# YihongSun/Dynamo-Depth

Hardware: AMD Instinct MI355X
Metric: training images/sec (192x640 triplets) (higher is better)
Workload: dtype f32

## Files before the change

dynamo-depth_amd/csrc/dd_conv_mfma.hip:

```cpp
#include <hip/hip_runtime.h>
#include <cstdlib>
#include <type_traits>

#include "../../include/dynamo_hip.h"
#include "dd_attr.h"
#include "dd_split.h"
#include "dd_store_tile.h"

namespace dd {
namespace cm {

constexpr int TH = 8, TW = 32, NT = 256;
constexpr int HH = TH + 2, HW = TW + 2, HN = HH * HW;
constexpr int CK = 16;
constexpr int PSTR = 48;
constexpr int A_PIECE = HN * PSTR;
constexpr int A_BYTES = 3 * A_PIECE;
__device__ __forceinline__ int halo_addr(int px, int half) {
  return px * 48 + half * 16;
}
__host__ __device__ constexpr int pieces_of(int products) { return products == 6 ? 3 : (products == 3 ? 2 : 1); }
constexpr int FRAG = 1024;
constexpr int PRE = (HN * 4 + NT - 1) / NT;

// ... 176 lines not shown
      if (tap == 1) fetch(min(chunk + 1, nchunks - 1));
      constexpr int PA[6] = {2, 0, 1, 1, 0, 0}, PB[6] = {0, 2, 1, 0, 1, 0};
#pragma unroll
      for (int t = 6 - NP; t < 6; ++t)
#pragma unroll
        for (int m = 0; m < 2; ++m)
#pragma unroll
          for (int n = 0; n < NB; ++n)
            acc[m][n] = __builtin_amdgcn_mfma_f32_32x32x16_bf16(__builtin_bit_cast(bf8, af[cur][m][PA[t]]), __builtin_bit_cast(bf8, bfr[cur][n][PB[t]]), acc[m][n], 0, 0, 0);
      __builtin_amdgcn_sched_barrier(0);
      if (tap < 8) {
        store_b(s + 2);
        lds_barrier();
      }
    }
  }

  auto tail = [&](auto full) {
#pragma unroll
    for (int n = 0; n < NB; ++n) {
      const int co = (ntile * NB + n) * 32 + (lane & 31);
#pragma unroll
      for (int m = 0; m < 2; ++m) {
        const int Y = Y0 + 2 * wave + m, X = X0 + 4 * (lane >> 5);
        float* p = y + (((size_t)b * Ho + Y) * Wo + X) * n_out + co;
        store_acc32<decltype(full)::value>(acc[m][n], bv[n], p, (size_t)n_out, (co < n_out && Y < Ho) ? Wo - X : 0, StoreF32{});
      }
    }
  };
  if (X0 + TW <= Wo && Y0 + TH <= Ho && (ntile + 1) * (32 * NB) <= n_out) tail(std::true_type{});
  else tail(std::false_type{});
}

constexpr int FLAT_MT = 256;
constexpr int FLAT_ZERO = HN - 1;
constexpr int FLAT_MAX_W = (FLAT_ZERO - FLAT_MT) / 2 - 1;

template <int NB, int NP>
__global__ __launch_bounds__(NT, 2) void conv_mfma_flat_kernel(const float* __restrict__ x, const uint4* __restrict__ pack, const float* __restrict__ bias,
                                                               int H, int W, int M, int k_in, int n_out, int splits, float* __restrict__ out) {
  extern __shared__ __align__(16) unsigned char smem[];
  unsigned char* const s_b = smem + A_BYTES;
  const int tid = threadIdx.x, lane = tid & 63, wave = __builtin_amdgcn_readfirstlane(tid >> 6);
  const int p0 = (int)blockIdx.x * FLAT_MT, ntile = blockIdx.y, split = blockIdx.z;
  const int nchunks = (k_in + CK - 1) / CK;
  const int c_begin = (int)((long long)nchunks * split / splits), c_end = (int)((long long)nchunks * (split + 1) / splits);
  const int win = FLAT_MT + 2 * (W + 1), q0 = p0 - (W + 1);
  const char* pk = reinterpret_cast<const char*>(pack) + (size_t)ntile * nchunks * 9 * (3 * NB * FRAG);

  int g_off[PRE], l_off[PRE];
#pragma unroll
  for (int j = 0; j < PRE; ++j) {
    const int i = tid + j * NT, px = i >> 2, q = i & 3;
    const int fp = q0 + px;
    l_off[j] = px < win ? halo_addr(px, q >> 1) + (q & 1) * 8 : -1;
    g_off[j] = (px < win && fp >= 0 && fp < M) ? fp * k_in + q * 4 : -1;
  }
  if (tid < 9) {
    const int pc = tid / 3, part = tid % 3;
    if (part * 16 < PSTR) *reinterpret_cast<uint4*>(smem + pc * A_PIECE + FLAT_ZERO * PSTR + part * 16) = make_uint4(0u, 0u, 0u, 0u);
  }
  float4 pre[PRE];
  auto fetch = [&](int chunk) {
#pragma unroll
    for (int j = 0; j < PRE; ++j) {
      const int c0 = chunk * CK + (((tid + j * NT) & 3) << 2);
// ... 136 lines not shown
    const float4 v = P[(size_t)s * total4 + i];
    a.x += v.x; a.y += v.y; a.z += v.z; a.w += v.w;
  }
  if (bias) {
    const int c = (i * 4) % n_out;
    a.x += bias[c]; a.y += bias[c + 1]; a.z += bias[c + 2]; a.w += bias[c + 3];
  }
  reinterpret_cast<float4*>(y)[i] = a;
}

static int flat_splits(int M, int k_in, int n_out) {
  const int wgs = ((M + FLAT_MT - 1) / FLAT_MT) * ((n_out + 63) / 64), nchunks = (k_in + CK - 1) / CK;
  const char* env = getenv("DD_FLAT_SPLITS");
  int s = env ? atoi(env) : (480 + wgs / 2) / wgs;
  if (s > nchunks / 2) s = nchunks / 2;
  return s < 1 ? 1 : s;
}

static size_t pack_bytes(int n_out, int k_in) { return (size_t)frags_of(n_out, k_in) * 3 * FRAG; }

template <int NB, int NP>
static int launch(const float* x, const void* pack, const float* bias, int B, int Hi, int Wi, int k_in, int n_out, int pad, float* y, hipStream_t stream) {
  const int Ho = Hi + 2 * pad - 2, Wo = Wi + 2 * pad - 2;
  const int tiles_x = (Wo + TW - 1) / TW, tiles_y = (Ho + TH - 1) / TH;
  auto kern = conv_mfma_kernel<NB, NP>;
  static dd::LdsAttrOnce lds_attr;
  if (const int rc = lds_attr.ensure(reinterpret_cast<const void*>(kern), (int)(lds_bytes<NB>()))) return rc;
  dim3 grid(tiles_x * tiles_y, (n_out + 32 * NB - 1) / (32 * NB), B);
  hipLaunchKernelGGL(kern, grid, dim3(NT), lds_bytes<NB>(), stream, x, static_cast<const uint4*>(pack), bias, Hi, Wi, Ho, Wo, k_in, n_out, pad, tiles_x,
                     tiles_y, y);
  return (int)hipGetLastError();
}

template <int NP>
static int launch_blocks(const float* x, const void* pack, const float* bias, int B, int Hi, int Wi, int k_in, int n_out, int pad, float* y, hipStream_t s) {
  switch (blocks_for(n_out)) {
    case 1: return launch<1, NP>(x, pack, bias, B, Hi, Wi, k_in, n_out, pad, y, s);
    case 2: return launch<2, NP>(x, pack, bias, B, Hi, Wi, k_in, n_out, pad, y, s);
    default: return launch<3, NP>(x, pack, bias, B, Hi, Wi, k_in, n_out, pad, y, s);
  }
}

template <int NP>
static int launch_flat(const float* x, const void* pack, const float* bias, int H, int W, int M, int k_in, int n_out, int splits, float* out, hipStream_t s) {
  auto kern = conv_mfma_flat_kernel<2, NP>;
  static dd::LdsAttrOnce lds_attr;
  if (const int rc = lds_attr.ensure(reinterpret_cast<const void*>(kern), (int)(lds_bytes<2>()))) return rc;
  hipLaunchKernelGGL(kern, dim3((M + FLAT_MT - 1) / FLAT_MT, (n_out + 63) / 64, splits), dim3(NT), lds_bytes<2>(), s, x, static_cast<const uint4*>(pack), bias, H, W, M, k_in,
                     n_out, splits, out);
  return (int)hipGetLastError();
}

namespace wg {
constexpr int TR = 2, TC = 16;
constexpr int XR = TR + 2, XC = TC + 2;
constexpr int XROW = 24;
constexpr int GSTR = TR * TC * 2 + 16;
constexpr int XSTR = XR * XROW * 2 + 16;
constexpr int G_PIECE = 64 * GSTR, X_PIECE = 64 * XSTR;
constexpr int LDS = 3 * (G_PIECE + X_PIECE);
constexpr int XITEMS = XR * (XC / 2) * 16;
constexpr int XJ = (XITEMS + NT - 1) / NT;
constexpr int BLOCK = 64 * 9 * 64;
}

template <int NP>
__global__ __launch_bounds__(NT, 2) void conv_wgrad_kernel(const float* __restrict__ x, const float* __restrict__ g, int B, int Hi, int Wi, int Ho, int Wo,
                                                           int cin, int cout, int pad, int tiles_x, int tiles_y, float* __restrict__ partial) {
// ... 205 lines not shown
extern "C" int dd_conv3x3_mfma_supported(int cin, int cout) {
  return (cin >= 16 && cout >= 16 && cin % 4 == 0 && cout % 4 == 0 && cin <= 1024 && cout <= 1024) ? 1 : 0;
}

extern "C" size_t dd_conv3x3_mfma_pack_bytes(int n_out, int k_in) { return dd::cm::pack_bytes(n_out, k_in); }

extern "C" int dd_conv3x3_mfma_pack(const float* weight, long long s_co, long long s_ci, long long s_kh, long long s_kw, int cout, int cin, void* pack_fwd,
                                    void* pack_bwd_data, void* stream) {
  using namespace dd::cm;
  if (!weight || (!pack_fwd && !pack_bwd_data) || cout < 1 || cin < 1) return (int)hipErrorInvalidValue;
  const int frags_fwd = pack_fwd ? (int)(pack_bytes(cout, cin) / (3 * FRAG)) : 0;
  const int frags_bwd = pack_bwd_data ? (int)(pack_bytes(cin, cout) / (3 * FRAG)) : 0;
  const int threads = (frags_fwd + frags_bwd) * 64;
  hipLaunchKernelGGL(conv_mfma_pack_kernel, dim3((threads + 255) / 256), dim3(256), 0, static_cast<hipStream_t>(stream), weight, s_co, s_ci, s_kh, s_kw, cout,
                     cin, static_cast<uint4*>(pack_fwd), static_cast<uint4*>(pack_bwd_data), frags_fwd, frags_bwd);
  return (int)hipGetLastError();
}

extern "C" int dd_conv3x3_mfma_pack_many_job_words(void) { return dd::cm::PACK_JOB_WORDS; }

extern "C" int dd_conv3x3_mfma_pack_many_blocks(int cout, int cin, int want_fwd, int want_bwd_data) {
  using namespace dd::cm;
  if (cout < 1 || cin < 1) return 0;
  return ((want_fwd ? frags_of(cout, cin) : 0) + (want_bwd_data ? frags_of(cin, cout) : 0) + 3) / 4;
}

extern "C" int dd_conv3x3_mfma_pack_many(const long long* jobs, const int* block_job, int n_blocks, void* stream) {
  using namespace dd::cm;
  if (!jobs || !block_job || n_blocks < 1) return (int)hipErrorInvalidValue;
  hipLaunchKernelGGL(conv_mfma_pack_many_kernel, dim3(n_blocks), dim3(256), 0, static_cast<hipStream_t>(stream), jobs, block_job);
  return (int)hipGetLastError();
}

extern "C" int dd_conv3x3_mfma_n(const float* x, const void* pack, const float* bias, int B, int Hi, int Wi, int k_in, int n_out, int pad, int products,
                                 float* y, void* stream) {
  using namespace dd::cm;
  if (!x || !pack || !y || B < 1 || pad < 0 || pad > 2 || Hi + 2 * pad < 3 || Wi + 2 * pad < 3 || k_in % 4 || k_in < 4 || n_out < 1) return (int)hipErrorInvalidValue;
  if ((size_t)Hi * Wi * k_in >= (1ull << 31) || (reinterpret_cast<unsigned long long>(x) & 15ull)) return (int)hipErrorInvalidValue;
  hipStream_t s = static_cast<hipStream_t>(stream);
  switch (products) {
    case 6: return launch_blocks<6>(x, pack, bias, B, Hi, Wi, k_in, n_out, pad, y, s);
    case 3: return launch_blocks<3>(x, pack, bias, B, Hi, Wi, k_in, n_out, pad, y, s);
    case 1: return launch_blocks<1>(x, pack, bias, B, Hi, Wi, k_in, n_out, pad, y, s);
    default: return (int)hipErrorInvalidValue;
  }
}

extern "C" int dd_conv3x3_mfma(const float* x, const void* pack, const float* bias, int B, int Hi, int Wi, int k_in, int n_out, int pad, float* y,
                               void* stream) {
  return dd_conv3x3_mfma_n(x, pack, bias, B, Hi, Wi, k_in, n_out, pad, 6, y, stream);
}

extern "C" int dd_conv3x3_mfma_flat_supported(int B, int H, int W, int k_in, int n_out) {
  using namespace dd::cm;
  return (B >= 1 && H >= 1 && W >= 1 && W <= FLAT_MAX_W && k_in >= 32 && k_in % 4 == 0 && k_in <= 1024 && n_out % 4 == 0 && n_out <= 1024 &&
          blocks_for(n_out) == 2 && n_out > 32 &&
          (size_t)B * H * W * (size_t)(k_in > n_out ? k_in : n_out) < (1ull << 31)) ? 1 : 0;
}

extern "C" size_t dd_conv3x3_mfma_flat_workspace_bytes(int B, int H, int W, int k_in, int n_out) {
  using namespace dd::cm;
  const int M = B * H * W, s = flat_splits(M, k_in, n_out);
  return s > 1 ? (size_t)s * M * n_out * sizeof(float) : 16;
}

extern "C" int dd_conv3x3_mfma_flat_n(const float* x, const void* pack, const float* bias, int B, int H, int W, int k_in, int n_out, int products, float* y,
                                      void* workspace, size_t workspace_bytes, void* stream) {
  using namespace dd::cm;
  if (!x || !pack || !y || !dd_conv3x3_mfma_flat_supported(B, H, W, k_in, n_out) || (reinterpret_cast<unsigned long long>(x) & 15ull) ||
      (reinterpret_cast<unsigned long long>(y) & 15ull) || (products != 6 && products != 3 && products != 1))
    return (int)hipErrorInvalidValue;
  const int M = B * H * W, splits = flat_splits(M, k_in, n_out);
  if (splits > 1 && (!workspace || workspace_bytes < dd_conv3x3_mfma_flat_workspace_bytes(B, H, W, k_in, n_out) || (reinterpret_cast<unsigned long long>(workspace) & 15ull)))
    return (int)hipErrorInvalidValue;
  hipStream_t s = static_cast<hipStream_t>(stream);
  float* out = splits > 1 ? static_cast<float*>(workspace) : y;
  const int rc = products == 6 ? launch_flat<6>(x, pack, bias, H, W, M, k_in, n_out, splits, out, s)
               : products == 3 ? launch_flat<3>(x, pack, bias, H, W, M, k_in, n_out, splits, out, s)
// ... 49 lines not shown
```

dynamo-depth_amd/hipops/abi.py:

```python
import ctypes as C

DD_MAX_SCALES = 4
DD_NUM_SRC = 2
DD_ABI_VERSION = 2
DD_MODE_RIGID, DD_MODE_FLOW, DD_MODE_FLOW_MASK = 0, 1, 2
DD_PARTIAL_STRIDE = 40
DD_SUMS_STRIDE = 8

_fp = C.c_void_p


class DDPhotoScale(C.Structure):
    _fields_ = [
        ("shift", C.c_int), ("h", C.c_int), ("w", C.c_int),
        ("w_photo", C.c_float), ("w_cons", C.c_float),
        ("disp", _fp),
        ("flow", _fp * DD_NUM_SRC),
        ("mask", _fp * DD_NUM_SRC),
        ("noise", _fp),
        ("g_disp", _fp),
        ("g_flow", _fp * DD_NUM_SRC),
        ("g_mask", _fp * DD_NUM_SRC),
        ("out_color", _fp * DD_NUM_SRC),
        ("out_sample", _fp * DD_NUM_SRC),
# ... 151 lines not shown
        "dd_layer_norm_bwd": (i, [v, v, v, v, v, C.c_longlong, i, v, v, v, z, v]),
        "dd_layer_norm_workspace_bytes": (z, [i]),
        "dd_layer_scale_bwd": (i, [v, v, v, i, i, i, v, v, v, z, v]),
        "dd_layer_scale_workspace_bytes": (z, [i, i]),
        "dd_layer_norm_fwd_t": (i, [v, C.c_longlong, i, v, v, f, v, v, v, i, v]),
        "dd_layer_norm_bwd_t": (i, [v, v, v, v, v, C.c_longlong, i, v, v, v, z, i, v]),
        "dd_layer_scale_bwd_t": (i, [v, v, v, i, i, i, v, v, v, z, i, v]),
        "dd_layer_scale_fwd_t": (i, [v, v, v, i, i, i, v, i, v]),
        "dd_dwconv3x3_nhwc_t": (i, [v, v, i, i, i, i, i, v, i, v]),
        "dd_dwconv3x3_nhwc_bwd_data_t": (i, [v, v, i, i, i, i, i, v, i, v]),
        "dd_dwconv3x3_nhwc_bwd_weight_t": (i, [v, v, i, i, i, i, i, v, v, z, i, v]),
        "dd_redu_supported": (i, [i, i]),
        "dd_redu_workspace_bytes": (z, [C.c_longlong, i, i]),
        "dd_redu_fwd": (i, [v, v, v, v, C.c_longlong, i, i, v, v]),
        "dd_redu_bwd_data": (i, [v, v, C.c_longlong, i, i, v, v, v]),
        "dd_redu_bwd_weight": (i, [v, v, v, C.c_longlong, i, i, v, v, v, z, v]),
        "dd_conv_head_supported": (i, [i]),
        "dd_conv_head_workspace_bytes": (z, [i, i, i, i]),
        "dd_conv_head_fwd": (i, [v, v, C.c_longlong, C.c_longlong, C.c_longlong, v, i, i, i, i, v, v]),
        "dd_conv_head_bwd_weight": (i, [v, v, i, i, i, i, v, v, v, z, v]),
        "dd_conv_small_supported": (i, [i, i, i]),
        "dd_conv_small_workspace_bytes": (z, [i, i, i]),
        "dd_conv_small_fwd": (i, [v, v, C.c_longlong, C.c_longlong, C.c_longlong, C.c_longlong, v, i, i, i, i, i, i, v, v, z, v]),
        "dd_conv_small_bwd_data": (i, [v, v, C.c_longlong, C.c_longlong, C.c_longlong, C.c_longlong, i, i, i, i, i, i, v, v, z, v]),
        "dd_conv_small_bwd_weight": (i, [v, v, i, i, i, i, i, i, v, v, v, z, v]),
        "dd_conv3x3_mfma_supported": (i, [i, i]),
        "dd_conv3x3_mfma_pack_bytes": (z, [i, i]),
        "dd_conv3x3_mfma_pack": (i, [v, C.c_longlong, C.c_longlong, C.c_longlong, C.c_longlong, i, i, v, v, v]),
        "dd_conv3x3_mfma_pack_many_job_words": (i, []),
        "dd_conv3x3_mfma_pack_many_blocks": (i, [i, i, i, i]),
        "dd_conv3x3_mfma_pack_many": (i, [v, v, i, v]),
        "dd_conv3x3_mfma": (i, [v, v, v, i, i, i, i, i, i, v, v]),
        "dd_conv3x3_mfma_n": (i, [v, v, v, i, i, i, i, i, i, i, v, v]),
        "dd_conv3x3_mfma_flat_supported": (i, [i, i, i, i, i]),
        "dd_conv3x3_mfma_flat_workspace_bytes": (z, [i, i, i, i, i]),
        "dd_conv3x3_mfma_flat": (i, [v, v, v, i, i, i, i, i, v, v, z, v]),
        "dd_conv3x3_mfma_flat_n": (i, [v, v, v, i, i, i, i, i, i, v, v, z, v]),
        "dd_conv3x3_mfma_wgrad_workspace_bytes": (z, [i, i, i, i, i]),
        "dd_conv3x3_mfma_bwd_weight": (i, [v, v, i, i, i, i, i, i, v, v, z, v]),
        "dd_conv3x3_mfma_bwd_weight_n": (i, [v, v, i, i, i, i, i, i, i, v, v, z, v]),
        "dd_conv3x3_half_supported": (i, [i, i]),
        "dd_conv3x3_half_pack_bytes": (z, [i, i]),
        "dd_conv3x3_half_pack": (i, [v, C.c_longlong, C.c_longlong, C.c_longlong, C.c_longlong, i, i, i, v, v, v]),
        "dd_conv3x3_half": (i, [v, v, v, i, i, i, i, i, i, i, v, v]),
        "dd_conv3x3_half_wgrad_workspace_bytes": (z, [i, i, i, i, i]),
        "dd_conv3x3_half_bwd_weight": (i, [v, v, i, i, i, i, i, i, i, v, v, z, v]),
        "dd_pw_gemm_pack_bytes": (z, [i, i]),
        "dd_mlp_pack": (i, [v, C.c_longlong, C.c_longlong, v, C.c_longlong, C.c_longlong, i, i, v, v, v, v, v, v]),
        "dd_mlp_fwd_supported": (i, [i]),
        "dd_mlp_fwd": (i, [v, v, v, v, v, i, i, v, v]),
        "dd_pw_gemm": (i, [v, v, v, i, i, i, i, v, v]),
        "dd_gelu_pair": (i, [v, v, v, z, v]),
        "dd_adam_chunk": (i, []),
        "dd_adam_multi": (i, [v, i, v, i, v, C.c_double, C.c_double, C.c_double, C.c_double, C.c_double, v, v, v]),
        "dd_error_string": (C.c_char_p, [i]),
        "dd_abi_version": (i, []),
    }
    found = []
    for name, (res, args) in sig.items():
        try:
            fn = getattr(lib, name)
        except AttributeError:
            continue
        fn.restype = res
        fn.argtypes = args
        found.append(name)
    return found


EXPORTED = (
    "dd_photo_loss", "dd_photo_workspace_bytes", "dd_photo_timing", "dd_photo_timing_read", "dd_photo_loss_part", "dd_smooth_loss", "dd_smooth_workspace_bytes",
    "dd_ground_loss", "dd_ground_workspace_bytes", "dd_ground_plane", "dd_ground_candidates", "dd_ground_select",
    "dd_assemble_losses", "dd_reg_losses_finish", "dd_fused_loss", "dd_fused_loss_part", "dd_fused_loss_supported", "dd_reg_workspace_bytes", "dd_backproject", "dd_backproject_bwd", "dd_project3d", "dd_project3d_bwd", "dd_project3d_workspace_bytes",
    "dd_ssim", "dd_ssim_bwd", "dd_disp_to_depth", "dd_pose_matrix", "dd_pose_matrix_bwd",
    "dd_channel_sum_nhwc", "dd_channel_sum_workspace_bytes", "dd_reflect_pad1_nhwc", "dd_reflect_pad1_nhwc_bwd",
    "dd_dwconv3x3_nhwc", "dd_dwconv3x3_nhwc_bwd_data", "dd_dwconv3x3_nhwc_bwd_weight", "dd_dwconv3x3_workspace_bytes", "dd_conv3x3_cout1_bwd_data",
    "dd_prepare_frames", "dd_prepare_frames_workspace_bytes", "dd_pyramid_down2", "dd_pack_rgb", "dd_depth_metrics", "dd_depth_metrics_workspace_bytes", "dd_depth_metrics_masked", "dd_depth_metrics_masked_workspace_bytes", "dd_motion_pr", "dd_fill_contours", "dd_vis_frame", "dd_vis_flow_tiles", "dd_bn_act_fwd", "dd_bn_act_bwd", "dd_bn_workspace_bytes",
    "dd_bn_act_fwd_t", "dd_bn_act_bwd_t", "dd_channel_sum_nhwc_t", "dd_reflect_pad1_nhwc_t", "dd_reflect_pad1_nhwc_bwd_t", "dd_up_cat_pad_t", "dd_up_cat_pad_bwd_t",
    "dd_layer_norm_fwd", "dd_layer_norm_bwd", "dd_layer_norm_workspace_bytes", "dd_layer_scale_bwd", "dd_layer_scale_workspace_bytes",
    "dd_jpeg_workspace_bytes", "dd_jpeg_decode", "dd_resize_workspace_bytes", "dd_resize_bicubic", "dd_layer_norm_fwd_t", "dd_layer_norm_bwd_t", "dd_layer_scale_bwd_t", "dd_layer_scale_fwd_t", "dd_dwconv3x3_nhwc_t", "dd_dwconv3x3_nhwc_bwd_data_t",
    "dd_dwconv3x3_nhwc_bwd_weight_t", "dd_adam_chunk", "dd_adam_multi", "dd_conv_small_supported", "dd_conv_small_workspace_bytes",
    "dd_conv_small_fwd", "dd_conv_small_bwd_data", "dd_conv_small_bwd_weight", "dd_conv_head_supported", "dd_conv_head_workspace_bytes", "dd_conv_head_fwd",
    "dd_conv_head_bwd_weight", "dd_redu_supported", "dd_redu_workspace_bytes", "dd_redu_fwd", "dd_redu_bwd_data", "dd_redu_bwd_weight",
    "dd_conv3x3_mfma_supported", "dd_conv3x3_mfma_pack_bytes", "dd_conv3x3_mfma_pack", "dd_conv3x3_mfma_pack_many_job_words",
    "dd_conv3x3_mfma_pack_many_blocks", "dd_conv3x3_mfma_pack_many", "dd_conv3x3_mfma", "dd_conv3x3_mfma_n",
    "dd_conv3x3_mfma_flat_supported", "dd_conv3x3_mfma_flat_workspace_bytes", "dd_conv3x3_mfma_flat", "dd_conv3x3_mfma_flat_n",
    "dd_conv3x3_mfma_wgrad_workspace_bytes", "dd_conv3x3_mfma_bwd_weight", "dd_conv3x3_mfma_bwd_weight_n",
    "dd_conv3x3_half_supported", "dd_conv3x3_half_pack_bytes", "dd_conv3x3_half_pack", "dd_conv3x3_half",
    "dd_conv3x3_half_wgrad_workspace_bytes", "dd_conv3x3_half_bwd_weight",
    "dd_pw_gemm_pack_bytes", "dd_mlp_pack", "dd_pw_gemm", "dd_gelu_pair", "dd_mlp_fwd_supported", "dd_mlp_fwd",
    "dd_error_string", "dd_abi_version",
)


def fill_photo_args(*, B, H, W, mode, automask, want_grad, min_depth, max_depth, ssim_weight, eps, disp_thr,
                    target, source, K, inv_K, T, ts, g_T, sums, workspace, scales, source_packed=None):
    a = DDPhotoArgs()
    a.abi_version = DD_ABI_VERSION
    a.B, a.H, a.W = B, H, W
    a.num_scales = len(scales)
    a.mode, a.automask, a.want_grad = mode, int(bool(automask)), int(bool(want_grad))
    a.min_depth, a.max_depth, a.ssim_weight, a.eps, a.disp_thr = min_depth, max_depth, ssim_weight, eps, disp_thr
    a.target = ptr(target)
    a.K, a.inv_K = ptr(K), ptr(inv_K)
    a.sums, a.workspace = ptr(sums), ptr(workspace)
    for f in range(DD_NUM_SRC):
        a.source[f] = ptr(source[f])
        a.source_packed[f] = ptr(source_packed[f]) if source_packed is not None else None
        a.T[f] = ptr(T[f])
        a.ts[f] = ptr(ts[f]) if ts is not None else None
        a.g_T[f] = ptr(g_T[f]) if g_T is not None else None
    for s, d in enumerate(scales):
        sc = a.scale[s]
        sc.shift, sc.h, sc.w = d["shift"], d["h"], d["w"]
        sc.w_photo, sc.w_cons = d.get("w_photo", 0.0), d.get("w_cons", 0.0)
        for name in ("disp", "noise", "g_disp", "out_depth", "out_idsel"):
            setattr(sc, name, ptr(d.get(name)))
        for name in ("flow", "mask", "g_flow", "g_mask", "out_color", "out_sample", "out_resid", "out_delta"):
# ... 6 lines not shown
```

dynamo-depth_amd/hipops/functions.py:

```python
import os

import torch

from . import lib as L
from .pack_many import PackSet, _ACTIVE_PACK_SETS, _pack_many_on, pack_many_launches, pack_weights_once_per_forward


def _dev(t, name="tensor"):
    if not t.is_cuda:
        raise L.DynamoHipError("%s must live on the GPU: the Dynamo-Depth loss path has no CPU implementation "
                               "(libdynamo_hip.so is the only backend)" % name)
    if t.dtype != torch.float32:
        raise L.DynamoHipError("%s must be float32, got %s" % (name, t.dtype))
    return t.contiguous()


DTYPE_CODE = {torch.float32: 0, torch.float16: 1, torch.bfloat16: 2}


def _p(t):
    return None if t is None else t.data_ptr()


def _ws(nbytes, device):
# ... 409 lines not shown
def mfma_conv_ok(x, weight, stride, padding, dilation, groups):
    if os.environ.get("DD_STOCK_MFMA_CONV", "0") == "1":
        return False
    if not (x.is_cuda and x.dtype == torch.float32 and weight.dtype == torch.float32 and x.dim() == 4):
        return False
    if not _conv3x3_s1(x, weight, stride, padding, dilation, groups, ((0, 0), (1, 1))) or torch.is_autocast_enabled():
        return False
    cout, cin = weight.shape[:2]
    pad = padding[0]
    Ho, Wo = x.shape[2] + 2 * pad - 2, x.shape[3] + 2 * pad - 2
    if _below_tile_pixels(x.shape[0], Ho, Wo, "DD_MFMA_CONV_MIN_PIXELS"):
        return pad == 1 and _flat_conv_ok(x.shape[0], x.shape[2], x.shape[3], cin, cout)
    return bool(L.load().dd_conv3x3_mfma_supported(cin, cout))


def _flat_conv_ok(B, H, W, cin, cout):
    if os.environ.get("DD_FLAT_MFMA_CONV", "1") != "1" or min(cin, cout) < int(os.environ.get("DD_FLAT_MIN_CHANNELS", "256")):
        return False
    lib = L.load()
    return bool(lib.dd_conv3x3_mfma_flat_supported(B, H, W, cin, cout)) and bool(lib.dd_conv3x3_mfma_flat_supported(B, H, W, cout, cin))


def _flat_shape(B, H, W, pad, k_in=None, n_out=None):
    Ho, Wo = H + 2 * pad - 2, W + 2 * pad - 2
    if not (pad == 1 and _below_tile_pixels(B, Ho, Wo, "DD_MFMA_CONV_MIN_PIXELS")):
        return False
    if os.environ.get("DD_FLAT_MFMA_CONV", "1") != "1":
        return False
    return k_in is None or bool(L.load().dd_conv3x3_mfma_flat_supported(B, H, W, k_in, n_out))


_MFMA_CONV_CALLS = [0]
_FLAT_CONV_CALLS = [0]


def mfma_conv_calls():
    return _MFMA_CONV_CALLS[0]


_PRODUCTS = {"highest": 6, "high": 3, "medium": 1}


def mfma_products():
    env = os.environ.get("DD_MFMA_PRODUCTS")
    return int(env) if env else _PRODUCTS[torch.get_float32_matmul_precision()]


class MfmaConvFn(torch.autograd.Function):

    @staticmethod
    def forward(ctx, x, weight, bias, pad):
        lib = L.load()
        cout, cin = weight.shape[:2]
        B, _, Hi, Wi = x.shape
        x = _dense_nhwc(x)
        need_gx = ctx.needs_input_grad[0]
        stream = L.current_stream()
        products = mfma_products()
        pset = _ACTIVE_PACK_SETS[-1] if (_ACTIVE_PACK_SETS and _pack_many_on()) else None
        packs = pset.take(weight, need_gx) if pset is not None else None
        if packs is not None:
            pack_f, pack_b = packs
        else:
            pack_f = torch.empty(_ws_bytes("dd_conv3x3_mfma_pack_bytes", cout, cin) // 4, dtype=torch.float32, device=x.device)
            pack_b = torch.empty(_ws_bytes("dd_conv3x3_mfma_pack_bytes", cin, cout) // 4, dtype=torch.float32, device=x.device) if need_gx else None
            sw = weight.stride()
            L.check(lib.dd_conv3x3_mfma_pack(_p(weight), sw[0], sw[1], sw[2], sw[3], cout, cin, _p(pack_f), _p(pack_b), stream), "dd_conv3x3_mfma_pack")
            if pset is not None and isinstance(weight, torch.nn.Parameter):
                pset.join(weight, pack_f, pack_b)
        Ho, Wo = Hi + 2 * pad - 2, Wi + 2 * pad - 2
        y = _nhwc_empty(B, cout, Ho, Wo, x.device)
        if _flat_shape(B, Hi, Wi, pad, cin, cout):
            nbytes = _ws_bytes("dd_conv3x3_mfma_flat_workspace_bytes", B, Hi, Wi, cin, cout)
            ws = _ws(nbytes, x.device)
            L.check(lib.dd_conv3x3_mfma_flat_n(_p(x), _p(pack_f), _p(bias), B, Hi, Wi, cin, cout, products, _p(y), _p(ws), nbytes, stream), "dd_conv3x3_mfma_flat")
            _FLAT_CONV_CALLS[0] += 1
        else:
            L.check(lib.dd_conv3x3_mfma_n(_p(x), _p(pack_f), _p(bias), B, Hi, Wi, cin, cout, pad, products, _p(y), stream), "dd_conv3x3_mfma")
        _MFMA_CONV_CALLS[0] += 1
        ctx.save_for_backward(x, weight, pack_b)
        ctx.conf = (pad, bias is not None, products)
        return y

    @staticmethod
    def backward(ctx, g):
        x, weight, pack_b = ctx.saved_tensors
        pad, has_bias, products = ctx.conf
        lib = L.load()
        cout, cin = weight.shape[:2]
        B, _, Hi, Wi = x.shape
        Ho, Wo = g.shape[2:]
        g = _dense_nhwc(g.to(torch.float32))
        gx = gw = gb = None
        stream = L.current_stream()
        if ctx.needs_input_grad[0]:
            gx = _nhwc_empty(B, cin, Hi, Wi, g.device)
            if _flat_shape(B, Hi, Wi, pad, cout, cin):
                nbytes = _ws_bytes("dd_conv3x3_mfma_flat_workspace_bytes", B, Ho, Wo, cout, cin)
                ws = _ws(nbytes, g.device)
                L.check(lib.dd_conv3x3_mfma_flat_n(_p(g), _p(pack_b), None, B, Ho, Wo, cout, cin, products, _p(gx), _p(ws), nbytes, stream), "dd_conv3x3_mfma_flat (data gradient)")
            else:
                L.check(lib.dd_conv3x3_mfma_n(_p(g), _p(pack_b), None, B, Ho, Wo, cout, cin, 2 - pad, products, _p(gx), stream), "dd_conv3x3_mfma (data gradient)")
        if ctx.needs_input_grad[1]:
            if (cout % 4 == 0 and min(cin, cout) >= 32 and os.environ.get("DD_STOCK_MFMA_WGRAD", "0") != "1"
                    and (products < 6 or not _flat_shape(B, Hi, Wi, pad, cin, cout))):
                flat = torch.empty(cout * 9 * cin, dtype=torch.float32, device=g.device)
                nbytes = _ws_bytes("dd_conv3x3_mfma_wgrad_workspace_bytes", B, Ho, Wo, cin, cout)
                ws = _ws(nbytes, g.device)
                L.check(lib.dd_conv3x3_mfma_bwd_weight_n(_p(x), _p(g), B, Hi, Wi, cin, cout, pad, products, _p(flat), _p(ws), nbytes, stream), "dd_conv3x3_mfma_bwd_weight")
                gw = flat.view(cout, 3, 3, cin).permute(0, 3, 1, 2)
            else:
                gw = _wgrad_3x3_library(g, x, weight, pad)
        if has_bias and ctx.needs_input_grad[2]:
            gb = _channel_sum(g, B * Ho * Wo, cout, DTYPE_CODE[g.dtype], stream) if cout <= 256 else g.sum((0, 2, 3))
        return gx, gw, gb, None


def mfma_conv(x, weight, bias=None, pad=1):
    return MfmaConvFn.apply(x, weight, bias, int(pad))


_HALF_CONV_CALLS = [0]


def half_conv_calls():
    return _HALF_CONV_CALLS[0]


def half_conv_ok(x, weight, stride, padding, dilation, groups):
    if os.environ.get("DD_HALF_MFMA_CONV", "1") != "1" or not x.is_cuda or x.dim() != 4 or x.dtype not in (torch.float16, torch.bfloat16):
        return False
    if not torch.is_autocast_enabled() or torch.get_autocast_dtype("cuda") != x.dtype or weight.dtype not in (torch.float32, x.dtype):
        return False
    if not _conv3x3_s1(x, weight, stride, padding, dilation, groups, ((0, 0), (1, 1))):
        return False
# ... 579 lines not shown
```

include/dynamo_hip.h:

```cpp
#ifndef DYNAMO_HIP_H_
#define DYNAMO_HIP_H_

#include <stddef.h>
#include <stdint.h>

#ifdef __cplusplus
extern "C" {
#endif

#define DD_MAX_SCALES 4
#define DD_NUM_SRC 2
#define DD_ABI_VERSION 2

#define DD_MODE_RIGID 0
#define DD_MODE_FLOW 1
#define DD_MODE_FLOW_MASK 2

#define DD_PARTIAL_STRIDE 40
#define DD_SUMS_STRIDE 8

typedef struct DDPhotoScale {
  int shift;
  int h, w;
  float w_photo;
// ... 238 lines not shown
int dd_dwconv3x3_nhwc_bwd_data_t(const void* g_out, const float* weight, int B, int H, int W, int C, int dilation, void* g_x, int dtype, void* stream);
int dd_dwconv3x3_nhwc_bwd_weight_t(const void* g_out, const void* x, int B, int H, int W, int C, int dilation, float* g_weight, void* workspace,
                                   size_t workspace_bytes, int dtype, void* stream);

int dd_redu_supported(int C, int cout);
size_t dd_redu_workspace_bytes(long long P, int C, int cout);
int dd_redu_fwd(const float* a, const float* b, const float* weight, const float* bias, long long P, int C, int cout, float* y, void* stream);
int dd_redu_bwd_data(const float* g_out, const float* weight, long long P, int C, int cout, float* g_a, float* g_b, void* stream);
int dd_redu_bwd_weight(const float* a, const float* b, const float* g_out, long long P, int C, int cout, float* g_weight, float* g_bias, void* workspace,
                       size_t workspace_bytes, void* stream);

int dd_conv_head_supported(int C);
size_t dd_conv_head_workspace_bytes(int B, int Hp, int Wp, int C);
int dd_conv_head_fwd(const float* x_padded, const float* weight, long long s_ci, long long s_kh, long long s_kw, const float* bias, int B, int Hp, int Wp,
                     int C, float* out, void* stream);
int dd_conv_head_bwd_weight(const float* x_padded, const float* g_out, int B, int Hp, int Wp, int C, float* g_weight, float* g_bias, void* workspace,
                            size_t workspace_bytes, void* stream);

int dd_conv_small_supported(int ks, int cin, int cout);
size_t dd_conv_small_workspace_bytes(int ks, int cin, int cout);
int dd_conv_small_fwd(const float* x, const float* weight, long long s_co, long long s_ci, long long s_kh, long long s_kw, const float* bias, int B, int H,
                      int W, int cin, int cout, int ks, float* y, void* workspace, size_t workspace_bytes, void* stream);
int dd_conv_small_bwd_data(const float* g_out, const float* weight, long long s_co, long long s_ci, long long s_kh, long long s_kw, int B, int H, int W, int cin,
                           int cout, int ks, float* g_x, void* workspace, size_t workspace_bytes, void* stream);
int dd_conv_small_bwd_weight(const float* x, const float* g_out, int B, int H, int W, int cin, int cout, int ks, float* g_weight, float* g_bias,
                             void* workspace, size_t workspace_bytes, void* stream);

int dd_conv3x3_mfma_supported(int cin, int cout);
size_t dd_conv3x3_mfma_pack_bytes(int n_out, int k_in);
int dd_conv3x3_mfma_pack(const float* weight, long long s_co, long long s_ci, long long s_kh, long long s_kw, int cout, int cin, void* pack_fwd,
                         void* pack_bwd_data, void* stream);
int dd_conv3x3_mfma_n(const float* x, const void* pack, const float* bias, int B, int Hi, int Wi, int k_in, int n_out, int pad, int products, float* y,
                      void* stream);
int dd_conv3x3_mfma_pack_many_job_words(void);
int dd_conv3x3_mfma_pack_many_blocks(int cout, int cin, int want_fwd, int want_bwd_data);
int dd_conv3x3_mfma_pack_many(const long long* jobs, const int* block_job, int n_blocks, void* stream);
int dd_conv3x3_mfma(const float* x, const void* pack, const float* bias, int B, int Hi, int Wi, int k_in, int n_out, int pad, float* y, void* stream);
int dd_conv3x3_mfma_flat_supported(int B, int H, int W, int k_in, int n_out);
size_t dd_conv3x3_mfma_flat_workspace_bytes(int B, int H, int W, int k_in, int n_out);
int dd_conv3x3_mfma_flat(const float* x, const void* pack, const float* bias, int B, int H, int W, int k_in, int n_out, float* y, void* workspace,
                         size_t workspace_bytes, void* stream);
int dd_conv3x3_mfma_flat_n(const float* x, const void* pack, const float* bias, int B, int H, int W, int k_in, int n_out, int products, float* y,
                           void* workspace, size_t workspace_bytes, void* stream);
size_t dd_conv3x3_mfma_wgrad_workspace_bytes(int B, int Ho, int Wo, int cin, int cout);
int dd_conv3x3_mfma_bwd_weight(const float* x, const float* g_out, int B, int Hi, int Wi, int cin, int cout, int pad, float* g_weight, void* workspace,
                               size_t workspace_bytes, void* stream);
int dd_conv3x3_mfma_bwd_weight_n(const float* x, const float* g_out, int B, int Hi, int Wi, int cin, int cout, int pad, int products, float* g_weight,
                                 void* workspace, size_t workspace_bytes, void* stream);

int dd_conv3x3_half_supported(int cin, int cout);
size_t dd_conv3x3_half_pack_bytes(int n_out, int k_in);
int dd_conv3x3_half_pack(const float* weight, long long s_co, long long s_ci, long long s_kh, long long s_kw, int cout, int cin, int dtype,
                         void* pack_fwd, void* pack_bwd_data, void* stream);
int dd_conv3x3_half(const void* x, const void* pack, const float* bias, int B, int Hi, int Wi, int k_in, int n_out, int pad, int dtype, void* y,
                    void* stream);
size_t dd_conv3x3_half_wgrad_workspace_bytes(int B, int Ho, int Wo, int cin, int cout);
int dd_conv3x3_half_bwd_weight(const void* x, const void* g_out, int B, int Hi, int Wi, int cin, int cout, int pad, int dtype, float* g_weight,
                               void* workspace, size_t workspace_bytes, void* stream);

size_t dd_pw_gemm_pack_bytes(int N, int K);
int dd_mlp_pack(const float* w1, long long s1_n, long long s1_k, const float* w2, long long s2_n, long long s2_k, int C, int hidden, void* pack_fwd1,
                void* pack_fwd2, void* pack_bwd2, void* pack_bwd1, void* pack_fwd2_fused, void* stream);
int dd_mlp_fwd_supported(int C);
int dd_mlp_fwd(const float* x, const void* pack_fwd1, const void* pack_fwd2_fused, const float* b1, const float* b2, int M, int C, float* y, void* stream);
int dd_pw_gemm(const float* x, const void* pack, const float* bias, int M, int K, int N, int gelu_in, float* y, void* stream);
int dd_gelu_pair(const float* pre, float* g_inout, float* post, size_t n, void* stream);
// ... 37 lines not shown
```

Measured before the change: 368.3.

## Add 8-wave 16-row MFMA conv kernel with wave-specialized pipelines and launch heuristic

Adds an 8-wave (512-thread) variant of the 3x3 MFMA conv that covers a 16-row tile, so each staged halo is reused by more output rows and there are fewer tile edges. The two halves of the workgroup run differently phased software pipelines, with the late waves at raised priority, and tiles are remapped across XCDs. A heuristic picks 8 or 4 waves from the workgroup count versus CUs and from whether Ho divides by 16, with an environment override. The cost is more LDS per workgroup, possibly lower occupancy, and a heuristic that may choose badly on some layer shapes.

Result: no change. 366.7 (-0.4%).

```diff
diff --git a/dynamo-depth_amd/csrc/dd_conv_mfma.hip b/dynamo-depth_amd/csrc/dd_conv_mfma.hip
--- a/dynamo-depth_amd/csrc/dd_conv_mfma.hip
+++ b/dynamo-depth_amd/csrc/dd_conv_mfma.hip
@@ -232,6 +232,206 @@
   else tail(std::false_type{});
 }
 
+namespace w8 {
+constexpr int TH = 16, NT = 512;
+constexpr int HH = TH + 2, HN = HH * HW;
+constexpr int A_PIECE = HN * PSTR, A_BYTES = 3 * A_PIECE;
+constexpr int PRE = (HN * 4 + NT - 1) / NT;
+template <int NB>
+constexpr int b_buf_bytes() { return 3 * NB * FRAG; }
+template <int NB>
+constexpr int lds_bytes() { return A_BYTES + 3 * b_buf_bytes<NB>(); }
+}
+
+template <int NB, int NP>
+__global__ __launch_bounds__(w8::NT, 2) void conv_mfma8_kernel(const float* __restrict__ x, const uint4* __restrict__ pack, const float* __restrict__ bias,
+                                                               int Hi, int Wi, int Ho, int Wo, int k_in, int n_out, int pad, int tiles_x, int tiles_y,
+                                                               float* __restrict__ y) {
+  using w8::PRE;
+  extern __shared__ __align__(16) unsigned char smem[];
+  unsigned char* const s_b = smem + w8::A_BYTES;
+  const int tid = threadIdx.x, lane = tid & 63, wave = __builtin_amdgcn_readfirstlane(tid >> 6);
+  const int b = blockIdx.z, ntile = blockIdx.y;
+  int tile = blockIdx.x;
+  {
+    const int ntiles = gridDim.x, xc = tile & 7, base = ntiles >> 3, extra = ntiles & 7;
+    tile = xc * base + min(xc, extra) + (tile >> 3);
+  }
+  const int X0 = (tile % tiles_x) * TW, Y0 = (tile / tiles_x) * w8::TH;
+  const int nchunks = (k_in + CK - 1) / CK;
+  const float* xb = x + (size_t)b * Hi * Wi * k_in;
+  const char* pk = reinterpret_cast<const char*>(pack) + (size_t)ntile * nchunks * 9 * (3 * NB * FRAG);
+
+  int g_off[PRE];
+  int l_off[PRE];
+#pragma unroll
+  for (int j = 0; j < PRE; ++j) {
+    const int i = tid + j * w8::NT, px = i >> 2, q = i & 3;
+    const int hy = px / HW, hx = px - hy * HW;
+    const int Y = Y0 - pad + hy, X = X0 - pad + hx;
+    l_off[j] = px < w8::HN ? halo_addr(px, q >> 1) + (q & 1) * 8 : -1;
+    g_off[j] = (px < w8::HN && Y >= 0 && Y < Hi && X >= 0 && X < Wi) ? (Y * Wi + X) * k_in + q * 4 : -1;
+  }
+  float4 pre[PRE];
+  auto fetch = [&](int chunk) {
+#pragma unroll
+    for (int j = 0; j < PRE; ++j) {
+      const int c0 = chunk * CK + (((tid + j * w8::NT) & 3) << 2);
+      const int off = (g_off[j] >= 0 && c0 < k_in) ? g_off[j] + chunk * CK : 0;
+      pre[j] = *reinterpret_cast<const float4*>(xb + off);
+    }
+  };
+  auto stage = [&](int chunk) {
+#pragma unroll
+    for (int j = 0; j < PRE; ++j) {
+      if (l_off[j] >= 0) {
+        const int c0 = chunk * CK + (((tid + j * w8::NT) & 3) << 2);
+        const bool in = g_off[j] >= 0 && c0 < k_in;
+        const float4 v = in ? pre[j] : make_float4(0.f, 0.f, 0.f, 0.f);
+        unsigned a1, a2, a3, b1, b2, b3;
+        split2(v.x, v.y, a1, a2, a3);
+        split2(v.z, v.w, b1, b2, b3);
+        *reinterpret_cast<uint2*>(smem + l_off[j]) = make_uint2(a1, b1);
+        if (pieces_of(NP) > 1) *reinterpret_cast<uint2*>(smem + w8::A_PIECE + l_off[j]) = make_uint2(a2, b2);
+        if (pieces_of(NP) > 2) *reinterpret_cast<uint2*>(smem + 2 * w8::A_PIECE + l_off[j]) = make_uint2(a3, b3);
+      }
+    }
+  };
+  constexpr int BR = (3 * NB + 7) / 8;
+  uint4 breg[BR];
+#pragma unroll
+  for (int r = 0; r < BR; ++r) breg[r] = make_uint4(0u, 0u, 0u, 0u);
+  int b_frag[BR];
+#pragma unroll
+  for (int r = 0; r < BR; ++r) b_frag[r] = wave + 8 * r < 3 * NB ? wave + 8 * r : 0;
+  auto fetch_b = [&](int s) {
+    const char* src = pk + (size_t)s * (3 * NB * FRAG) + lane * 16;
+#pragma unroll
+    for (int r = 0; r < BR; ++r) breg[r] = *reinterpret_cast<const uint4*>(src + b_frag[r] * FRAG);
+  };
+  auto store_b = [&](int slot) {
+    unsigned char* dst = s_b + slot * w8::b_buf_bytes<NB>() + lane * 16;
+#pragma unroll
+    for (int r = 0; r < BR; ++r) *reinterpret_cast<uint4*>(dst + b_frag[r] * FRAG) = breg[r];
+  };
+  auto lds_barrier = [&]() { asm volatile("s_waitcnt lgkmcnt(0)\n\ts_barrier" ::: "memory"); };
+
+  f16v acc[2][NB];
+#pragma unroll
+  for (int m = 0; m < 2; ++m)
+#pragma unroll
+    for (int n = 0; n < NB; ++n)
+#pragma unroll
+      for (int r = 0; r < 16; ++r) acc[m][n][r] = 0.f;
+
+  const int a_pix = (2 * wave) * HW + (lane & 31), a_half = lane >> 5;
+  const unsigned char* b_lane = s_b + lane * 16;
+  uint4 af[2][2][3], bfr[2][NB][3];
+  auto read_a = [&](int set, int tap) {
+    const int ty = tap / 3, tx = tap % 3;
+#pragma unroll
+    for (int m = 0; m < 2; ++m) {
+      const unsigned char* ap = smem + halo_addr(a_pix + (m + ty) * HW + tx, a_half);
+#pragma unroll
+      for (int pc = 0; pc < pieces_of(NP); ++pc) af[set][m][pc] = *reinterpret_cast<const uint4*>(ap + pc * w8::A_PIECE);
+    }
+  };
+  auto read_b = [&](int set, int slot) {
+    const unsigned char* bb = b_lane + slot * w8::b_buf_bytes<NB>();
+#pragma unroll
+    for (int n = 0; n < NB; ++n)
+#pragma unroll
+      for (int pc = 0; pc < pieces_of(NP); ++pc) bfr[set][n][pc] = *reinterpret_cast<const uint4*>(bb + (n * 3 + pc) * FRAG);
+  };
+  auto read_frags = [&](int set, int tap, int slot) {
+    read_a(set, tap);
+    read_b(set, slot);
+  };
+  auto mfmas = [&](int cur) {
+    constexpr int PA[6] = {2, 0, 1, 1, 0, 0}, PB[6] = {0, 2, 1, 0, 1, 0};
+#pragma unroll
+    for (int t = 6 - NP; t < 6; ++t)
+#pragma unroll
+      for (int m = 0; m < 2; ++m)
+#pragma unroll
+        for (int n = 0; n < NB; ++n)
+          acc[m][n] = __builtin_amdgcn_mfma_f32_32x32x16_bf16(__builtin_bit_cast(bf8, af[cur][m][PA[t]]), __builtin_bit_cast(bf8, bfr[cur][n][PB[t]]), acc[m][n], 0, 0, 0);
+  };
+
+  const int nsteps = nchunks * 9;
+  const bool late = wave >= 4;
+  float bv[NB];
+#pragma unroll
+  for (int n = 0; n < NB; ++n) bv[n] = tile_bias(bias, (ntile * NB + n) * 32 + (lane & 31), n_out, pack);
+  fetch_b(0);
+  fetch(0);
+  store_b(0);
+  fetch_b(1);
+  if (late) __builtin_amdgcn_s_setprio(1);
+  if (!late) {
+    for (int chunk = 0; chunk < nchunks; ++chunk) {
+      stage(chunk);
+      store_b(1);
+      lds_barrier();
+      read_frags(0, 0, 0);
+#pragma unroll
+      for (int tap = 0; tap < 9; ++tap) {
+        const int s = chunk * 9 + tap, cur = tap & 1;
+        if (tap < 8) read_frags(cur ^ 1, tap + 1, (tap + 1) % 3);
+        fetch_b(min(s + 2, nsteps - 1));
+        if (tap == 1) fetch(min(chunk + 1, nchunks - 1));
+        mfmas(cur);
+        __builtin_amdgcn_sched_barrier(0);
+        if (tap < 8) {
+          store_b((tap + 2) % 3);
+          lds_barrier();
+        }
+      }
+    }
+  } else {
+    for (int chunk = 0; chunk < nchunks; ++chunk) {
+      stage(chunk);
+      store_b(1);
+      fetch_b(min(chunk * 9 + 2, nsteps - 1));
+      __builtin_amdgcn_sched_barrier(0);
+      read_b(1, 2);
+      if (chunk > 0) mfmas(1);
+      __builtin_amdgcn_sched_barrier(0);
+      lds_barrier();
+#pragma unroll
+      for (int tap = 0; tap < 8; ++tap) {
+        const int s = chunk * 9 + tap;
+        read_frags(0, tap, tap % 3);
+        store_b((tap + 2) % 3);
+        fetch_b(min(s + 3, nsteps - 1));
+        if (tap == 1) fetch(min(chunk + 1, nchunks - 1));
+        __builtin_amdgcn_sched_barrier(0);
+        mfmas(0);
+        if (tap == 7) read_a(1, 8);
+        __builtin_amdgcn_sched_barrier(0);
+        lds_barrier();
+      }
+    }
+    read_b(1, 2);
+    mfmas(1);
+  }
+
+  auto tail = [&](auto full) {
+#pragma unroll
+    for (int n = 0; n < NB; ++n) {
+      const int co = (ntile * NB + n) * 32 + (lane & 31);
+#pragma unroll
+      for (int m = 0; m < 2; ++m) {
+        const int Y = Y0 + 2 * wave + m, X = X0 + 4 * (lane >> 5);
+        float* p = y + (((size_t)b * Ho + Y) * Wo + X) * n_out + co;
+        store_acc32<decltype(full)::value>(acc[m][n], bv[n], p, (size_t)n_out, (co < n_out && Y < Ho) ? Wo - X : 0, StoreF32{});
+      }
+    }
+  };
+  if (X0 + TW <= Wo && Y0 + w8::TH <= Ho && (ntile + 1) * (32 * NB) <= n_out) tail(std::true_type{});
+  else tail(std::false_type{});
+}
+
 constexpr int FLAT_MT = 256;
 constexpr int FLAT_ZERO = HN - 1;
 constexpr int FLAT_MAX_W = (FLAT_ZERO - FLAT_MT) / 2 - 1;
@@ -434,8 +634,41 @@
   return (int)hipGetLastError();
 }
 
+template <int NB, int NP>
+static int launch8(const float* x, const void* pack, const float* bias, int B, int Hi, int Wi, int k_in, int n_out, int pad, float* y, hipStream_t stream) {
+  const int Ho = Hi + 2 * pad - 2, Wo = Wi + 2 * pad - 2;
+  const int tiles_x = (Wo + TW - 1) / TW, tiles_y = (Ho + w8::TH - 1) / w8::TH;
+  auto kern = conv_mfma8_kernel<NB, NP>;
+  static dd::LdsAttrOnce lds_attr;
+  if (const int rc = lds_attr.ensure(reinterpret_cast<const void*>(kern), (int)(w8::lds_bytes<NB>()))) return rc;
+  dim3 grid(tiles_x * tiles_y, (n_out + 32 * NB - 1) / (32 * NB), B);
+  hipLaunchKernelGGL(kern, grid, dim3(w8::NT), w8::lds_bytes<NB>(), stream, x, static_cast<const uint4*>(pack), bias, Hi, Wi, Ho, Wo, k_in, n_out, pad, tiles_x,
+                     tiles_y, y);
+  return (int)hipGetLastError();
+}
+
+static int waves_rule(int B, int Ho, int Wo, int k_in, int n_out) {
+  (void)k_in;
+  const int NB = blocks_for(n_out);
+  if (NB < 2 || Ho % w8::TH != 0) return 4;
+  const int cus = 256;
+  const int wgs = ((Wo + TW - 1) / TW) * (Ho / w8::TH) * ((n_out + 32 * NB - 1) / (32 * NB)) * B;
+  if (wgs <= cus) return 8;
+  const int last = wgs % cus;
+  return (NB == 2 && wgs > 2 * cus && (last == 0 || last >= (3 * cus) / 4)) ? 8 : 4;
+}
+
 template <int NP>
-static int launch_blocks(const float* x, const void* pack, const float* bias, int B, int Hi, int Wi, int k_in, int n_out, int pad, float* y, hipStream_t s) {
+static int launch_blocks(const float* x, const void* pack, const float* bias, int B, int Hi, int Wi, int k_in, int n_out, int pad, int waves, float* y,
+                         hipStream_t s) {
+  if (waves == 0) waves = waves_rule(B, Hi + 2 * pad - 2, Wi + 2 * pad - 2, k_in, n_out);
+  if (waves == 8) {
+    switch (blocks_for(n_out)) {
+      case 1: return launch8<1, NP>(x, pack, bias, B, Hi, Wi, k_in, n_out, pad, y, s);
+      case 2: return launch8<2, NP>(x, pack, bias, B, Hi, Wi, k_in, n_out, pad, y, s);
+      default: return launch8<3, NP>(x, pack, bias, B, Hi, Wi, k_in, n_out, pad, y, s);
+    }
+  }
   switch (blocks_for(n_out)) {
     case 1: return launch<1, NP>(x, pack, bias, B, Hi, Wi, k_in, n_out, pad, y, s);
     case 2: return launch<2, NP>(x, pack, bias, B, Hi, Wi, k_in, n_out, pad, y, s);
@@ -707,18 +940,26 @@
   return (int)hipGetLastError();
 }
 
-extern "C" int dd_conv3x3_mfma_n(const float* x, const void* pack, const float* bias, int B, int Hi, int Wi, int k_in, int n_out, int pad, int products,
-                                 float* y, void* stream) {
+extern "C" int dd_conv3x3_mfma_waves_rule(int B, int Ho, int Wo, int k_in, int n_out) { return dd::cm::waves_rule(B, Ho, Wo, k_in, n_out); }
+
+extern "C" int dd_conv3x3_mfma_waves(const float* x, const void* pack, const float* bias, int B, int Hi, int Wi, int k_in, int n_out, int pad, int products,
+                                     int waves, float* y, void* stream) {
   using namespace dd::cm;
   if (!x || !pack || !y || B < 1 || pad < 0 || pad > 2 || Hi + 2 * pad < 3 || Wi + 2 * pad < 3 || k_in % 4 || k_in < 4 || n_out < 1) return (int)hipErrorInvalidValue;
   if ((size_t)Hi * Wi * k_in >= (1ull << 31) || (reinterpret_cast<unsigned long long>(x) & 15ull)) return (int)hipErrorInvalidValue;
+  if (waves != 0 && waves != 4 && waves != 8) return (int)hipErrorInvalidValue;
   hipStream_t s = static_cast<hipStream_t>(stream);
   switch (products) {
-    case 6: return launch_blocks<6>(x, pack, bias, B, Hi, Wi, k_in, n_out, pad, y, s);
-    case 3: return launch_blocks<3>(x, pack, bias, B, Hi, Wi, k_in, n_out, pad, y, s);
-    case 1: return launch_blocks<1>(x, pack, bias, B, Hi, Wi, k_in, n_out, pad, y, s);
+    case 6: return launch_blocks<6>(x, pack, bias, B, Hi, Wi, k_in, n_out, pad, waves, y, s);
+    case 3: return launch_blocks<3>(x, pack, bias, B, Hi, Wi, k_in, n_out, pad, waves, y, s);
+    case 1: return launch_blocks<1>(x, pack, bias, B, Hi, Wi, k_in, n_out, pad, waves, y, s);
     default: return (int)hipErrorInvalidValue;
   }
+}
+
+extern "C" int dd_conv3x3_mfma_n(const float* x, const void* pack, const float* bias, int B, int Hi, int Wi, int k_in, int n_out, int pad, int products,
+                                 float* y, void* stream) {
+  return dd_conv3x3_mfma_waves(x, pack, bias, B, Hi, Wi, k_in, n_out, pad, products, 0, y, stream);
 }
 
 extern "C" int dd_conv3x3_mfma(const float* x, const void* pack, const float* bias, int B, int Hi, int Wi, int k_in, int n_out, int pad, float* y,
diff --git a/dynamo-depth_amd/hipops/abi.py b/dynamo-depth_amd/hipops/abi.py
--- a/dynamo-depth_amd/hipops/abi.py
+++ b/dynamo-depth_amd/hipops/abi.py
@@ -207,6 +207,8 @@
         "dd_conv3x3_mfma_pack_many": (i, [v, v, i, v]),
         "dd_conv3x3_mfma": (i, [v, v, v, i, i, i, i, i, i, v, v]),
         "dd_conv3x3_mfma_n": (i, [v, v, v, i, i, i, i, i, i, i, v, v]),
+        "dd_conv3x3_mfma_waves_rule": (i, [i, i, i, i, i]),
+        "dd_conv3x3_mfma_waves": (i, [v, v, v, i, i, i, i, i, i, i, i, v, v]),
         "dd_conv3x3_mfma_flat_supported": (i, [i, i, i, i, i]),
         "dd_conv3x3_mfma_flat_workspace_bytes": (z, [i, i, i, i, i]),
         "dd_conv3x3_mfma_flat": (i, [v, v, v, i, i, i, i, i, v, v, z, v]),
@@ -259,6 +261,7 @@
     "dd_conv_head_bwd_weight", "dd_redu_supported", "dd_redu_workspace_bytes", "dd_redu_fwd", "dd_redu_bwd_data", "dd_redu_bwd_weight",
     "dd_conv3x3_mfma_supported", "dd_conv3x3_mfma_pack_bytes", "dd_conv3x3_mfma_pack", "dd_conv3x3_mfma_pack_many_job_words",
     "dd_conv3x3_mfma_pack_many_blocks", "dd_conv3x3_mfma_pack_many", "dd_conv3x3_mfma", "dd_conv3x3_mfma_n",
+    "dd_conv3x3_mfma_waves_rule", "dd_conv3x3_mfma_waves",
     "dd_conv3x3_mfma_flat_supported", "dd_conv3x3_mfma_flat_workspace_bytes", "dd_conv3x3_mfma_flat", "dd_conv3x3_mfma_flat_n",
     "dd_conv3x3_mfma_wgrad_workspace_bytes", "dd_conv3x3_mfma_bwd_weight", "dd_conv3x3_mfma_bwd_weight_n",
     "dd_conv3x3_half_supported", "dd_conv3x3_half_pack_bytes", "dd_conv3x3_half_pack", "dd_conv3x3_half",
diff --git a/dynamo-depth_amd/hipops/functions.py b/dynamo-depth_amd/hipops/functions.py
--- a/dynamo-depth_amd/hipops/functions.py
+++ b/dynamo-depth_amd/hipops/functions.py
@@ -465,6 +465,15 @@
 
 _MFMA_CONV_CALLS = [0]
 _FLAT_CONV_CALLS = [0]
+_WAVES8_CALLS = [0]
+
+
+def _tile_waves(B, Ho, Wo, k_in, n_out):
+    env = os.environ.get("DD_MFMA_CONV_WAVES")
+    waves = int(env) if env else _ws_bytes("dd_conv3x3_mfma_waves_rule", B, Ho, Wo, k_in, n_out)
+    if waves == 8:
+        _WAVES8_CALLS[0] += 1
+    return waves
 
 
 def mfma_conv_calls():
@@ -509,7 +518,8 @@
             L.check(lib.dd_conv3x3_mfma_flat_n(_p(x), _p(pack_f), _p(bias), B, Hi, Wi, cin, cout, products, _p(y), _p(ws), nbytes, stream), "dd_conv3x3_mfma_flat")
             _FLAT_CONV_CALLS[0] += 1
         else:
-            L.check(lib.dd_conv3x3_mfma_n(_p(x), _p(pack_f), _p(bias), B, Hi, Wi, cin, cout, pad, products, _p(y), stream), "dd_conv3x3_mfma")
+            L.check(lib.dd_conv3x3_mfma_waves(_p(x), _p(pack_f), _p(bias), B, Hi, Wi, cin, cout, pad, products, _tile_waves(B, Ho, Wo, cin, cout), _p(y), stream),
+                    "dd_conv3x3_mfma")
         _MFMA_CONV_CALLS[0] += 1
         ctx.save_for_backward(x, weight, pack_b)
         ctx.conf = (pad, bias is not None, products)
@@ -533,7 +543,8 @@
                 ws = _ws(nbytes, g.device)
                 L.check(lib.dd_conv3x3_mfma_flat_n(_p(g), _p(pack_b), None, B, Ho, Wo, cout, cin, products, _p(gx), _p(ws), nbytes, stream), "dd_conv3x3_mfma_flat (data gradient)")
             else:
-                L.check(lib.dd_conv3x3_mfma_n(_p(g), _p(pack_b), None, B, Ho, Wo, cout, cin, 2 - pad, products, _p(gx), stream), "dd_conv3x3_mfma (data gradient)")
+                L.check(lib.dd_conv3x3_mfma_waves(_p(g), _p(pack_b), None, B, Ho, Wo, cout, cin, 2 - pad, products, _tile_waves(B, Hi, Wi, cout, cin), _p(gx),
+                                                  stream), "dd_conv3x3_mfma (data gradient)")
         if ctx.needs_input_grad[1]:
             if (cout % 4 == 0 and min(cin, cout) >= 32 and os.environ.get("DD_STOCK_MFMA_WGRAD", "0") != "1"
                     and (products < 6 or not _flat_shape(B, Hi, Wi, pad, cin, cout))):
diff --git a/include/dynamo_hip.h b/include/dynamo_hip.h
--- a/include/dynamo_hip.h
+++ b/include/dynamo_hip.h
@@ -294,6 +294,9 @@
                          void* pack_bwd_data, void* stream);
 int dd_conv3x3_mfma_n(const float* x, const void* pack, const float* bias, int B, int Hi, int Wi, int k_in, int n_out, int pad, int products, float* y,
                       void* stream);
+int dd_conv3x3_mfma_waves_rule(int B, int Ho, int Wo, int k_in, int n_out);
+int dd_conv3x3_mfma_waves(const float* x, const void* pack, const float* bias, int B, int Hi, int Wi, int k_in, int n_out, int pad, int products,
+                          int waves, float* y, void* stream);
 int dd_conv3x3_mfma_pack_many_job_words(void);
 int dd_conv3x3_mfma_pack_many_blocks(int cout, int cin, int want_fwd, int want_bwd_data);
 int dd_conv3x3_mfma_pack_many(const long long* jobs, const int* block_job, int n_blocks, void* stream);
```
